# lhoangan/arap_flow

Measured on AMD Instinct MI355X. Metric: ARAP solve+warp frames/sec at 854x480 mesh, higher is better.
Workload: dtype f32; 1 GPU; configs[1]: single 854x480 DAVIS-shaped frame, single-segment mask, fd=1; schedule 19/8/400; segments_per_frame=1, fd=1, parallelism=frames sharded, no collective, grid_vertices_per_frame=409920

## Files before the change

arap_flow_amd/csrc/arap_resident.h:

```cpp
#pragma once
#include <type_traits>
#include "arap_device.h"

namespace arap {

constexpr int RES_WGS = 512;
constexpr int RES_MAX_GROUPS = 16;
constexpr int RES_THREADS = 256;
constexpr int RES_SLOTS = 9;
constexpr int RES_TILES_PER_WG = RES_SLOTS;
constexpr int RT_X = 32, RT_Y = 8;
constexpr int RES_ZX = 2 * RT_X + 2 * RT_Y;
constexpr int RES_ZG = 2 * RES_ZX;
constexpr int RES_MAX_L = 32000;
static_assert(RT_X * RT_Y == RES_THREADS && RT_Y == 2 * (RES_THREADS / 64), "one vertex per lane, two rows per wavefront");
constexpr int RES_MAX_HALO = RES_TILES_PER_WG * (2 * RT_X + 2 * RT_Y);
constexpr int RES_HALO_PER_THREAD = (RES_MAX_HALO + RES_THREADS - 1) / RES_THREADS;
constexpr int RES_MAX_TILES = RES_WGS * RES_TILES_PER_WG;
constexpr int LROW = RT_X + 2;
constexpr int LROWS = RT_Y + 2;
constexpr int LPLANE = LROW * LROWS;
constexpr int LTILE = 5 * LPLANE;
constexpr int RES_LDS_BYTES = RES_TILES_PER_WG * LTILE * 4
                              + ((RES_MAX_HALO * 8 + 15) / 16) * 16
                              + RES_TILES_PER_WG * 8 + 8 + 384
                              + RES_TILES_PER_WG * RES_ZX * 16;
static_assert(2 * ((RES_LDS_BYTES + 1279) / 1280 * 1280) <= 160 * 1024, "two workgroups per CU");
#ifndef RES_HALO_REG_SLOTS
#define RES_HALO_REG_SLOTS 8
#endif
#ifndef RES_WREG_SLOTS
#define RES_WREG_SLOTS 7
#endif
#ifndef RES_WREG_8
#define RES_WREG_8 2
#endif
#ifndef RES_WREG_9
#define RES_WREG_9 2
#endif
#ifndef RES_WREG_FIT
#define RES_WREG_FIT 6
#endif
#ifndef RES_WREG_FIT_FLAT
#define RES_WREG_FIT_FLAT 7
#endif
#ifndef RES_WREG_8_FLAT
#define RES_WREG_8_FLAT 3
#endif
#ifndef RES_WREG_9_FLAT
#define RES_WREG_9_FLAT RES_WREG_9
#endif
#ifndef RES_FIRST_LOOK
#define RES_FIRST_LOOK 5
#endif
#ifndef RES_FIRST_LOOK_2
#define RES_FIRST_LOOK_2 14
#endif
#ifndef RES_FIRST_LOOK_X
#define RES_FIRST_LOOK_X 20
#endif
#ifndef RES_OWN_LOCAL
#define RES_OWN_LOCAL 1
#endif
#ifndef RES_POLL_SLEEP
#define RES_POLL_SLEEP 1
#endif
constexpr unsigned RES_SPIN_LIMIT = 1u << 18;
#ifndef RES_GRAN_STRIDE
#define RES_GRAN_STRIDE 2
#endif
constexpr int RES_GS = RES_GRAN_STRIDE;
constexpr int RES_GRAN_UNITS = 2 * RES_WGS;
constexpr int RES_GRAN_L1 = 2 * RES_GRAN_UNITS * RES_GS;
constexpr int RES_GRAN2_STRIDE = 16;
constexpr int RES_GRAN2_GROUP = 2 * 8 * RES_GRAN2_STRIDE;
constexpr int RES_GRAN_X = RES_GRAN_L1 + 4 * RES_GRAN2_GROUP;
constexpr int RES_GRAN_PER_LAUNCH = RES_GRAN_X + RES_GRAN_L1;
#ifndef RES_FLAT_MAX_RUNS
#define RES_FLAT_MAX_RUNS 2
#endif

constexpr int RES_SUMS_ANY = 0, RES_SUMS_FLAT = 1, RES_SUMS_COUNT = 2;

struct ResWg {
    int slot;
    int rank;
    int wgs;
    int gran;
};

struct ResDev {
    const int* tilelist;
    const int* ntiles;
    const int* tilepos;
    const int* bandx0;
    unsigned long long* zx;
    int rtX, rtY;
    unsigned long long* gran;
    unsigned* err;
    const ResWg* wgmap;
    int allow_fast;
    int force_fail;
    int flat_runs;
    int nowait;
    int fuse_update;
    unsigned long long* stamps;
};

typedef __attribute__((address_space(1))) unsigned long long gu64;
typedef __attribute__((address_space(1))) unsigned gu32;

__device__ __forceinline__ int border_entry(int x, int y)
{
    return y == 0 ? x : (y == RT_Y - 1 ? RT_X + x : (x == 0 ? 2 * RT_X + y : (x == RT_X - 1 ? 2 * RT_X + RT_Y + y : -1)));
}
__device__ __forceinline__ void st_tagged(unsigned long long* p, unsigned hi , float v, bool fast)
{
    const unsigned long long g = ((unsigned long long)hi << 32) | __float_as_uint(v);
    if (fast) __hip_atomic_store(p, g, __ATOMIC_RELAXED, __HIP_MEMORY_SCOPE_WORKGROUP);
    else __hip_atomic_store(p, g, __ATOMIC_RELAXED, __HIP_MEMORY_SCOPE_AGENT);
}
typedef float v2f_t __attribute__((ext_vector_type(2)));
__device__ __forceinline__ float2 fma2(float2 a, float2 b, float2 c)
{
    const v2f_t r = __builtin_elementwise_fma((v2f_t){a.x, a.y}, (v2f_t){b.x, b.y}, (v2f_t){c.x, c.y});
    return make_float2(r.x, r.y);
}
template <int BITNO>
__device__ __forceinline__ float keep_if(unsigned f, float v)
{
    int m;
    asm("v_bfe_i32 %0, %1, %2, 1" : "=v"(m) : "v"(f), "n"(BITNO));
    return __uint_as_float(__float_as_uint(v) & (unsigned)m);
}

__device__ __forceinline__ double block_sum_uniform(double t)
{
    return __hiloint2double(__builtin_amdgcn_readlane(__double2hiint(t), 3), __builtin_amdgcn_readlane(__double2loint(t), 3));
}

__device__ __forceinline__ bool group_sum(double part, unsigned epoch, unsigned long long* gran_group, int rank,
                                          int wgs, float* bcast , unsigned* err, float& out,
                                          bool fast = false, double* out_d = nullptr, bool nowait = false,
                                          unsigned long long* tm = nullptr ,
                                          unsigned long long* tarr = nullptr )
{
    const int wave = threadIdx.x >> 6, lane = threadIdx.x & 63;
    unsigned long long c0 = 0ull, c1;
    if (wave == 0) {
        if (tm) c0 = __builtin_amdgcn_s_memtime();
        if (tarr) *tarr += __builtin_amdgcn_s_memrealtime();
        __builtin_amdgcn_s_setprio(3);
        unsigned long long* buf = gran_group + (size_t)(epoch & 1u) * wgs * RES_GS;
        if ((lane >> 1) == 1) {
            const unsigned long long bits = (unsigned long long)__double_as_longlong(part);
            const unsigned hw = lane == 2 ? (unsigned)bits : (unsigned)(bits >> 32);
            const unsigned long long gv = ((unsigned long long)epoch << 32) | hw;
            if (fast)
                __hip_atomic_store(buf + rank * RES_GS + (lane - 2), gv, __ATOMIC_RELAXED, __HIP_MEMORY_SCOPE_WORKGROUP);
            else
                __hip_atomic_store(buf + rank * RES_GS + (lane - 2), gv, __ATOMIC_RELAXED, __HIP_MEMORY_SCOPE_AGENT);
        }
        part = block_sum_uniform(part);
        double v = 0.0;
        bool ok = false;
        if (tm) { c1 = __builtin_amdgcn_s_memtime(); tm[0] += c1 - c0; c0 = c1; }
        __builtin_amdgcn_s_sleep(RES_FIRST_LOOK);
        for (unsigned spins = 0; spins < RES_SPIN_LIMIT; ++spins) {
            if (tm) tm[3] += 1;
            v = 0.0;
            bool mine_ok = true;
            for (int m = lane; m < wgs; m += 64) {
                const unsigned long long lo = __hip_atomic_load(buf + RES_GS * m, __ATOMIC_RELAXED, __HIP_MEMORY_SCOPE_AGENT);
                const unsigned long long hi =
                    __hip_atomic_load(buf + RES_GS * m + 1, __ATOMIC_RELAXED, __HIP_MEMORY_SCOPE_AGENT);
                const bool own = RES_OWN_LOCAL && m == rank;
                mine_ok = mine_ok && (own || ((unsigned)(lo >> 32) == epoch && (unsigned)(hi >> 32) == epoch));
                v += own ? part : __longlong_as_double((long long)((hi << 32) | (lo & 0xffffffffull)));
            }
            ok = __all(mine_ok) || nowait;
            if (ok) break;
            if (RES_POLL_SLEEP) __builtin_amdgcn_s_sleep(1);
        }
        if (tm) { c1 = __builtin_amdgcn_s_memtime(); tm[1] += c1 - c0; c0 = c1; asm volatile("" : "+v"(v)); }
        v = wave_sum_l63_full(v);
        if (tm) {
            asm volatile("" :: "v"(v));
            c1 = __builtin_amdgcn_s_memtime(); tm[4] += c1 - c0;
        }
        if (lane == 63) {
            *(float2*)(bcast + 2 * (epoch & 1u)) = make_float2((float)v, ok ? 1.0f : 0.0f);
            if (out_d) *out_d = v;
            if (!ok) atomicExch(err, 0xDEAD0000u | (epoch & 0xffffu));
        }
        __builtin_amdgcn_s_setprio(0);
        if (tm) { c1 = __builtin_amdgcn_s_memtime(); tm[2] += c1 - c0; c0 = c1; }
    }
    __syncthreads();
    const float2 bc = *(const float2*)(bcast + 2 * (epoch & 1u));
    out = bc.x;
    if (tm && wave == 0) {
        asm volatile("s_waitcnt lgkmcnt(0)" ::: "memory");
        tm[5] += __builtin_amdgcn_s_memtime() - c0;
    }
    return bc.y != 0.0f;
}

__device__ __forceinline__ bool group_sum_h(double part, unsigned epoch, unsigned long long* gran_group,
                                            unsigned long long* gran2 , int rank, int wgs,
                                            float* bcast, unsigned* err, float& out, bool subfast)
{
    const int wave = threadIdx.x >> 6, lane = threadIdx.x & 63;
    if (wave == 0) {
        __builtin_amdgcn_s_setprio(3);
        const int sub = rank >> 6, srank = rank & 63, nsub = wgs >> 6;
        unsigned long long* buf = gran_group + (size_t)sub * (128 * RES_GS) + (size_t)(epoch & 1u) * (64 * RES_GS);
        part = __hiloint2double(__builtin_amdgcn_readfirstlane(__double2hiint(part)),
                                __builtin_amdgcn_readfirstlane(__double2loint(part)));
        if (lane < 2) {
            const unsigned long long bits = (unsigned long long)__double_as_longlong(part);
            const unsigned hw = lane == 0 ? (unsigned)bits : (unsigned)(bits >> 32);
            const unsigned long long gv = ((unsigned long long)epoch << 32) | hw;
// ... 100 lines not shown
        v = wave_sum_l63_full(v);
        if (lane == 63) {
            *(float2*)(bcast + 2 * (epoch & 1u)) = make_float2((float)v, ok ? 1.0f : 0.0f);
            if (!ok) atomicExch(err, 0xDEAD4000u | (epoch & 0x3fffu));
        }
        __builtin_amdgcn_s_setprio(0);
    }
    __syncthreads();
    const float2 bc = *(const float2*)(bcast + 2 * (epoch & 1u));
    out = bc.x;
    return bc.y != 0.0f;
}

__device__ __forceinline__ void halo_append(bool take, unsigned short val, unsigned short* hlist, int* nhalo)
{
    const unsigned long long m = __ballot(take);
    if (m == 0ull) return;
    const int first = __builtin_ctzll(m);
    int base = 0;
    if ((int)(threadIdx.x & 63) == first) base = atomicAdd(nhalo, __popcll(m));
    base = __builtin_amdgcn_readlane(base, first);
    const int before = (int)__builtin_amdgcn_mbcnt_hi((unsigned)(m >> 32), __builtin_amdgcn_mbcnt_lo((unsigned)m, 0u));
    if (take) hlist[base + before] = val;
}

__device__ __forceinline__ double block_sum8(double v, double* wsum ,
                                             unsigned long long* tb = nullptr )
{
    static_assert(RES_THREADS / 64 == 4, "one pair sum and one DPP step add four wavefronts");
    unsigned long long c0 = 0ull, c1;
    if (tb) { c0 = __builtin_amdgcn_s_memtime(); asm volatile("" : "+v"(v)); }
    v = wave_sum_l63_full(v);
    if (tb) { asm volatile("" :: "v"(v)); c1 = __builtin_amdgcn_s_memtime(); tb[0] += c1 - c0; c0 = c1; }
    const int wave = threadIdx.x >> 6, lane = threadIdx.x & 63;
    if (lane == 63) wsum[wave] = v;
    __syncthreads();
    double t = 0.0;
    if (wave == 0) {
        const double a = wsum[lane & 3], b = wsum[(lane & 3) ^ 1];
        if (tb) { asm volatile("s_waitcnt lgkmcnt(0)" ::: "memory"); c1 = __builtin_amdgcn_s_memtime(); tb[1] += c1 - c0; c0 = c1; }
        t = dpp_add_f64_full<0x112, 0xf>(a + b);
        if (tb) { asm volatile("" :: "v"(t)); c1 = __builtin_amdgcn_s_memtime(); tb[2] += c1 - c0; }
    }
    return t;
}

template <bool STAMPS, int NS, int SUMS>
__global__ __launch_bounds__(RES_THREADS, 2) void k_pcg_resident(PlanDev pd, ResDev rd, int L)
{
    static_assert(NS >= 1 && NS <= RES_SLOTS, "slots");
    static_assert(SUMS == RES_SUMS_ANY || SUMS == RES_SUMS_FLAT, "group-sum flavour");
    constexpr bool FLAT = SUMS == RES_SUMS_FLAT;
    constexpr bool SPEND = FLAT && !STAMPS;
    constexpr int WFIT = SPEND ? RES_WREG_FIT_FLAT : RES_WREG_FIT;
    unsigned long long tA = 0, tS1 = 0, tB = 0, tS2 = 0, tU = 0, t0 = 0, t1 = 0;
    unsigned long long tm[6] = {0, 0, 0, 0, 0, 0}, tbs = 0, tzr = 0;
    unsigned long long tbp[3] = {0, 0, 0}, tarr[2] = {0, 0};
#define RES_STAMP(acc) do { if (STAMPS) { t1 = __builtin_amdgcn_s_memrealtime(); acc += t1 - t0; t0 = t1; } } while (0)
    extern __shared__ __attribute__((aligned(16))) float lds[];
    const ResWg me = rd.wgmap[blockIdx.x];
    if (me.slot < 0) return;
    const int rank = me.rank;
    if (rd.force_fail) {
        if (threadIdx.x == 0) atomicExch(rd.err, 0xDEADFFFFu);
        return;
    }
    if (__hip_atomic_load(rd.err, __ATOMIC_RELAXED, __HIP_MEMORY_SCOPE_AGENT) != 0u) return;
    const int b = me.slot;
    const int wgs = me.wgs;
    const int W = pd.W, H = pd.H;
    const size_t gb = (size_t)b * pd.N;
    const int tid = threadIdx.x, lane = tid & 63, wave = tid >> 6;
    const int lx = lane & (RT_X - 1), ly = (wave << 1) | (lane >> 5);
    unsigned short* hlist = (unsigned short*)(lds + RES_TILES_PER_WG * LTILE);
    int2* tbase = (int2*)((char*)hlist + ((RES_MAX_HALO * 8 + 15) / 16) * 16);
    float* moLUT = (float*)(tbase + RES_TILES_PER_WG + 1);
    float* bcast = moLUT + 12;
    int* nhalo = (int*)(bcast + 4);
    double* wsum = (double*)(bcast + 6);
    unsigned* nbits = (unsigned*)(wsum + 10);
    unsigned* nremote = nbits + 16;
    float4* zst = (float4*)((char*)lds + RES_LDS_BYTES - RES_TILES_PER_WG * RES_ZX * 16);
    unsigned long long* gran_group = rd.gran + me.gran;
    unsigned long long* granx_group = FLAT ? nullptr : rd.gran + RES_GRAN_X + me.gran;

    const int nt = rd.ntiles[b];
    const int tbase_n = nt / wgs, textra = nt - tbase_n * wgs;
    const int tp = tbase_n + (rank < textra ? 1 : 0);
    const int tfirst = rank * tbase_n + (rank < textra ? rank : textra);
    const int* tl = rd.tilelist + (size_t)b * RES_MAX_TILES;
    float wr2, wf2;
    {
        const Slot sl = pd.slots[b];
        wr2 = sl.wr * sl.wr;
        wf2 = sl.wf * sl.wf;
        if (tid < 10) {
            const int deg = tid % 5, fit = tid / 5;
            float dO = 0.f;
            for (int k = 0; k < deg; ++k) dO = dO + (sl.wr * sl.wr + sl.wr * sl.wr);
            if (fit) dO = fmaf(sl.wf, sl.wf, dO);
            moLUT[tid] = ginv(dO);
        }
        if (tid == 0) { *nhalo = 0; *nremote = 0u; }
        if (tid < 16) nbits[tid] = 0u;
    }

    float rx[NS], ry[NS], ra[NS];
    float dx_[NS], dy_[NS], da_[NS];
    float apx[NS], apy[NS], apa[NS];
    float ma_[NS], mo_[NS];
    unsigned fl[NS];
    int ibase[NS];
    constexpr int NWR = NS <= RES_WREG_SLOTS ? 4 : (NS == 8 ? (SPEND ? RES_WREG_8_FLAT : RES_WREG_8)
                                                            : (SPEND ? RES_WREG_9_FLAT : RES_WREG_9));
    constexpr bool WREG = NWR > 0;
    float we[WREG ? NS : 1][5];
    const int loff = lx + W * ly;

    const int cell = (ly + 1) * LROW + (lx + 1);
#define TP2(T) ((float2*)(T))
#define TCS(T) ((float2*)(T) + LPLANE)
#define TPA(T) ((T) + 4 * LPLANE)

    int org_[NS];
#pragma unroll
    for (int j = 0; j < NS; ++j) org_[j] = j < tp ? tl[tfirst + j] : -1;
    unsigned long long* const zx_b = rd.zx + (size_t)b * RES_MAX_TILES * RES_ZG;
    for (int c = tid; c < tp * RES_ZG; c += RES_THREADS)
        __hip_atomic_store(zx_b + (size_t)tfirst * RES_ZG + c, 0ull, __ATOMIC_RELAXED, __HIP_MEMORY_SCOPE_AGENT);
    float2 qC[NS], qR[NS], vR[NS], vC[NS], hR[NS], hC[NS];
    float qRa[NS], qM[NS], vRa[NS], vM[NS], hRa[NS], hM[NS];
    unsigned qF[NS], vF[NS], hF[NS];
    const int vrow = ly == 0 ? 0 : RT_Y + 1, hcol = lx == 0 ? 0 : RT_X + 1;
#pragma unroll
    for (int j = 0; j < NS; ++j) {
        qC[j] = qR[j] = vR[j] = vC[j] = hR[j] = hC[j] = make_float2(0.f, 0.f);
        qRa[j] = qM[j] = vRa[j] = vM[j] = hRa[j] = hM[j] = 0.f;
        qF[j] = vF[j] = hF[j] = 0u;
        const int org = org_[j];
        const int y0 = org / W, x0 = org - y0 * W;
        const int x = x0 + lx, y = y0 + ly;
        if (org >= 0 && x < W && y < H) {
            const size_t i = gb + (size_t)(x + W * y);
            qF[j] = pd.flags[i];
            qC[j] = pd.cs[i];
            qR[j] = pd.rO[i]; qRa[j] = pd.rA[i]; qM[j] = pd.preA[i];
            if ((ly == 0 && y0 > 0) || (ly == RT_Y - 1 && y + 1 < H)) {
                const size_t hi = ly == 0 ? i - W : i + W;
                vF[j] = pd.flags[hi]; vR[j] = pd.rO[hi]; vRa[j] = pd.rA[hi]; vM[j] = pd.preA[hi]; vC[j] = pd.cs[hi];
            }
            if ((lx == 0 && x0 > 0) || (lx == RT_X - 1 && x + 1 < W)) {
                const size_t hi = lx == 0 ? i - 1 : i + 1;
                hF[j] = pd.flags[hi]; hR[j] = pd.rO[hi]; hRa[j] = pd.rA[hi]; hM[j] = pd.preA[hi]; hC[j] = pd.cs[hi];
            }
        }
    }
    for (int c = tid; c < NS * LTILE; c += RES_THREADS) lds[c] = 0.f;
    __syncthreads();
#pragma unroll
    for (int j = 0; j < NS; ++j) {
        dx_[j] = dy_[j] = da_[j] = 0.f;
        apx[j] = apy[j] = apa[j] = 0.f;
        const int org = org_[j];
        int x0 = -1, y0 = -1;
        if (org >= 0) { y0 = org / W; x0 = org - y0 * W; }
        float* T = lds + j * LTILE;
        const bool act = (qF[j] & F_ACT) != 0u;
        rx[j] = act ? qR[j].x : 0.f; ry[j] = act ? qR[j].y : 0.f; ra[j] = act ? qRa[j] : 0.f;
        ma_[j] = act ? qM[j] : 0.f;
        mo_[j] = moLUT[__popc(qF[j] & 15u) + 5 * (int)((qF[j] >> 4) & 1u)];
        if (act) {
            TP2(T)[cell] = make_float2(mo_[j] * rx[j], mo_[j] * ry[j]);
            TCS(T)[cell] = qC[j];
            TPA(T)[cell] = ma_[j] * ra[j];
        }
        if (vF[j] & F_ACT) {
            const int hc = vrow * LROW + (lx + 1);
            const float mo = moLUT[__popc(vF[j] & 15u) + 5 * (int)((vF[j] >> 4) & 1u)];
            TP2(T)[hc] = make_float2(mo * vR[j].x, mo * vR[j].y); TCS(T)[hc] = vC[j]; TPA(T)[hc] = vM[j] * vRa[j];
        }
        if (hF[j] & F_ACT) {
            const int hc = (ly + 1) * LROW + hcol;
            const float mo = moLUT[__popc(hF[j] & 15u) + 5 * (int)((hF[j] >> 4) & 1u)];
            TP2(T)[hc] = make_float2(mo * hR[j].x, mo * hR[j].y); TCS(T)[hc] = hC[j]; TPA(T)[hc] = hM[j] * hRa[j];
        }
        fl[j] = qF[j];
        ibase[j] = __builtin_amdgcn_readfirstlane(x0 + W * y0);
        if (tid == 0) tbase[j] = make_int2(x0, y0);
    }
    float rho = read_scalar(pd.red + ((size_t)b * pd.nslots + 0) * NSHARD);
    __syncthreads();
#pragma unroll
    for (int j = 0; j < NS; ++j) {
        const unsigned f = fl[j];
        if (WREG) {
            if (NWR > 0) we[j][0] = keep_if<0>(f, wr2);
            if (NWR > 1) we[j][1] = keep_if<1>(f, wr2);
            if (NWR > 2) we[j][2] = keep_if<2>(f, wr2);
            if (NWR > 3) we[j][3] = keep_if<3>(f, wr2);
            if (NS <= WFIT) we[j][4] = keep_if<4>(f, wf2);
        }
        halo_append(ly == 0 && (f & F_E3), (unsigned short)(j * LPLANE + 0 * LROW + lx + 1), hlist, nhalo);
        halo_append(ly == RT_Y - 1 && (f & F_E2), (unsigned short)(j * LPLANE + (RT_Y + 1) * LROW + lx + 1), hlist, nhalo);
        halo_append(lx == 0 && (f & F_E1), (unsigned short)(j * LPLANE + (ly + 1) * LROW + 0), hlist, nhalo);
        halo_append(lx == RT_X - 1 && (f & F_E0), (unsigned short)(j * LPLANE + (ly + 1) * LROW + RT_X + 1), hlist, nhalo);
    }
    __syncthreads();
    const int nh = *nhalo;
    uint2* htab = (uint2*)hlist;
    constexpr bool HREG = NS <= RES_HALO_REG_SLOTS;
    uint2 hreg[RES_HALO_PER_THREAD];
    {
        uint2 e[RES_HALO_PER_THREAD];
#pragma unroll
        for (int u = 0; u < RES_HALO_PER_THREAD; ++u) {
            const int c = tid + u * RES_THREADS;
            e[u] = make_uint2(0u, 0u);
            if (c < nh) {
                const int id = hlist[c];
                const int k = id / LPLANE, rem = id - k * LPLANE;
                const int row = rem / LROW, col = rem - row * LROW;
                const int2 tb = tbase[k];
                const int gx = tb.x + col - 1, gy = tb.y + row - 1;
                e[u].y = (unsigned)(k * (LTILE / 2) + rem) | ((unsigned)(k * LTILE + 4 * LPLANE + rem) << 16);
                const int band = gy / RT_Y;
                const int kx = (gx - rd.bandx0[(size_t)b * rd.rtY + band]) / RT_X;
                const int pos = rd.tilepos[((size_t)b * rd.rtY + band) * rd.rtX + (kx < 0 ? 0 : (kx < rd.rtX ? kx : rd.rtX - 1))];
                const int nfull = textra * (tbase_n + 1);
                const int owner = pos < nfull ? pos / (tbase_n + 1) : textra + (pos - nfull) / (tbase_n > 0 ? tbase_n : 1);
                if (pos >= 0 && owner != rank) atomicOr(&nbits[(owner >> 5) & 15], 1u << (owner & 31));
                const int kxc = kx < 0 ? 0 : (kx < rd.rtX ? kx : rd.rtX - 1);
                const int lxo = gx - (rd.bandx0[(size_t)b * rd.rtY + band] + kxc * RT_X), lyo = gy - band * RT_Y;
                const int zpos = border_entry(lxo, lyo);
                (void)row; (void)col;
                e[u].x = (unsigned)((pos < 0 ? 0 : pos) * RES_ZG + 2 * zpos);
            }
        }
        __syncthreads();
#pragma unroll
        for (int u = 0; u < RES_HALO_PER_THREAD; ++u) {
            if (tid + u * RES_THREADS < RES_MAX_HALO) htab[tid + u * RES_THREADS] = e[u];
            hreg[u] = e[u];
        }
    }
    static_assert(RES_TILES_PER_WG * LTILE < 65536 && LTILE % 2 == 0, "halo table packs 16-bit cell offsets");

    unsigned offP[5], offA[5];
    {
        const int dn[5] = {0, 1, -1, LROW, -LROW};
#pragma unroll
        for (int n = 0; n < 5; ++n) {
            offP[n] = (unsigned)(cell + dn[n]) * 8u;
            offA[n] = (unsigned)(cell + dn[n]) * 4u;
            asm volatile("" : "+v"(offP[n]));
            asm volatile("" : "+v"(offA[n]));
        }
    }
    const int zent = border_entry(lx, ly);
    bool alive = true;
    float alpha_last = 0.f;
    asm volatile("s_waitcnt vmcnt(0)" ::: "memory");
    __syncthreads();
    bool fast = false, zfast = false;
    bool hier = false, subfast = false;
    bool hierx = false;
    unsigned long long* const gran2 =
        FLAT ? nullptr : rd.gran + RES_GRAN_L1 + ((((int)(blockIdx.x & 7u) - (me.rank >> 6)) >> 1) & 3) * RES_GRAN2_GROUP;
    {
        const unsigned xcc = __builtin_amdgcn_s_getreg((3 << 11) | (0 << 6) | 20) & 15u;
        float dummy;
        const double mine = (double)xcc + 65536.0 * (double)(xcc * xcc);
        alive = group_sum(mine, 1u, gran_group, rank, wgs, bcast, rd.err, dummy, false, wsum + 8);
        const double tot = wsum[8];
        const double s2 = floor(tot / 65536.0), s1 = tot - 65536.0 * s2;
        fast = rd.allow_fast && ((double)wgs * s2 == s1 * s1);
        __syncthreads();
        hier = !FLAT && !fast && wgs > 64;
        hierx = hier && (((wgs + 63) >> 6) <= 2 || ((wgs + 63) >> 6) <= rd.flat_runs);
        if (!fast && rd.allow_fast && alive) {
            if (wave == 0) {
                const unsigned long long* buf = gran_group + (size_t)1 * wgs * RES_GS;
                bool remote = false, elsewhere = false;
                for (int m = lane; m < wgs; m += 64) {
                    const bool nb = ((nbits[(m >> 5) & 15] >> (m & 31)) & 1u) != 0u;
                    const bool same_run = hier && (m >> 6) == (rank >> 6);
                    if (nb || same_run) {
                        const unsigned long long lo = __hip_atomic_load(buf + RES_GS * m, __ATOMIC_RELAXED, __HIP_MEMORY_SCOPE_AGENT);
                        const unsigned long long hi = __hip_atomic_load(buf + RES_GS * m + 1, __ATOMIC_RELAXED, __HIP_MEMORY_SCOPE_AGENT);
                        const double val = __longlong_as_double((long long)((hi << 32) | (lo & 0xffffffffull)));
                        const double q2 = floor(val / 65536.0);
                        const bool other = (unsigned)(lo >> 32) != 1u || (unsigned)(hi >> 32) != 1u ||
                                           (unsigned)(val - 65536.0 * q2) != xcc;
                        remote = remote || (nb && other);
                        elsewhere = elsewhere || (same_run && other);
                    }
                }
                const unsigned any_remote = __any(remote) ? 1u : 0u, any_elsewhere = __any(elsewhere) ? 2u : 0u;
                if (lane == 0) *nremote = any_remote | any_elsewhere;
            }
            __syncthreads();
            zfast = (*nremote & 1u) == 0u;
            subfast = !FLAT && hier && (*nremote & 2u) == 0u;
        } else {
            zfast = fast;
        }
        __syncthreads();
    }
#ifndef RES_PRIO_HI
#define RES_PRIO_HI 2
#endif
#ifndef RES_PRIO_TAIL
#define RES_PRIO_TAIL 2
#endif
#define RES_PRIO(J) { if ((J) + RES_PRIO_TAIL >= NS) __builtin_amdgcn_s_setprio(0); else __builtin_amdgcn_s_setprio(RES_PRIO_HI); }
#define RES_PRIO_END() __builtin_amdgcn_s_setprio(0);
    if (STAMPS) t0 = __builtin_amdgcn_s_memrealtime();
    for (int l = 0; l < L && alive; ++l) {
        static_assert(F_E0 == 1u && F_E1 == 2u && F_E2 == 4u && F_E3 == 8u && F_FIT == 16u && F_ACT == 32u, "bit numbers below");
        double acc = 0.0;
        float2 Lpv[2], Lcs[2], LqO[2][4], Lcn[2][4];
        float Lpa[2], LqA[2][4];
#define RES_LOAD_A(J)                                                                                  \
        {                                                                                              \
            const int s_ = (J) & 1;                                                                    \
            const char* T_ = (const char*)lds + (J) * (LTILE * 4);                                     \
            Lpv[s_] = *(const float2*)(T_ + offP[0]);                                                  \
            Lcs[s_] = *(const float2*)(T_ + offP[0] + LPLANE * 8);                                     \
            Lpa[s_] = *(const float*)(T_ + offA[0] + LPLANE * 16);                                     \
            _Pragma("unroll") for (int n_ = 0; n_ < 2; ++n_) {                                         \
                LqO[s_][n_] = *(const float2*)(T_ + offP[n_ + 1]);                                     \
                Lcn[s_][n_] = *(const float2*)(T_ + offP[n_ + 1] + LPLANE * 8);                        \
                LqA[s_][n_] = *(const float*)(T_ + offA[n_ + 1] + LPLANE * 16);                        \
            }                                                                                          \
        }
#define RES_LOAD_B(J)                                                                                  \
        {                                                                                              \
            const int s_ = (J) & 1;                                                                    \
            const char* T_ = (const char*)lds + (J) * (LTILE * 4);                                     \
            _Pragma("unroll") for (int n_ = 2; n_ < 4; ++n_) {                                         \
                LqO[s_][n_] = *(const float2*)(T_ + offP[n_ + 1]);                                     \
                Lcn[s_][n_] = *(const float2*)(T_ + offP[n_ + 1] + LPLANE * 8);                        \
                LqA[s_][n_] = *(const float*)(T_ + offA[n_ + 1] + LPLANE * 16);                        \
            }                                                                                          \
        }
        RES_LOAD_A(0)
        RES_LOAD_B(0)
#pragma unroll
        for (int j = 0; j < NS; ++j) {
            RES_PRIO(j)
            unsigned f = fl[j];
            asm volatile("" : "+v"(f));
            const int sj = j & 1;
            if (j + 1 < NS) RES_LOAD_A(j + 1)
            __builtin_amdgcn_sched_barrier(0);
            {
                const float2 pv = Lpv[sj];
                const float2 csv = Lcs[sj];
                const float pa_ = Lpa[sj];
                const float ci = csv.x, si = csv.y;
                const float2 pa2 = make_float2(pa_, pa_);
                float2 axy = make_float2(0.f, 0.f);
                float aa = 0.f;
#define RES_EDGE(BITNO, E, NQX, NQY, NHX, NHY, QX, QY)                                                 \
                {                                                                                      \
                    const float2 qO = LqO[sj][E], cn2 = Lcn[sj][E];                                    \
                    const float qA = LqA[sj][E];                                                       \
                    const float cn = cn2.x, sn = cn2.y;                                                \
                    const float w = (BITNO < NWR) ? we[WREG ? j : 0][BITNO] : keep_if<BITNO>(f, wr2);  \
                    const float2 e = pv - qO;                                                          \
                    const float2 t = fma2(make_float2(NQX, NQY), pa2, e);                              \
                    const float2 u = fma2(make_float2(NHX, NHY), make_float2(qA, qA), e + t);          \
                    axy = fma2(make_float2(w, w), u, axy);                                             \
                    aa = fmaf(-w, fmaf(QX, t.x, (QY) * t.y), aa);                                      \
                    (void)cn; (void)sn;                                                                \
                }
                RES_EDGE(0, 0,     -si,  ci,   -sn,  cn,    si, -ci)
                RES_EDGE(1, 1,      si, -ci,    sn, -cn,   -si,  ci)
                __builtin_amdgcn_sched_barrier(0);
                if (j + 1 < NS) RES_LOAD_B(j + 1)
                __builtin_amdgcn_sched_barrier(0);
                RES_EDGE(2, 2,     -ci, -si,   -cn, -sn,    ci,  si)
                RES_EDGE(3, 3,      ci,  si,    cn,  sn,   -ci, -si)
#undef RES_EDGE
                {
                    const float wf = (WREG && NS <= WFIT) ? we[WREG ? j : 0][4] : keep_if<4>(f, wf2);
                    axy = fma2(make_float2(wf, wf), pv, axy);
                }
                const float ax = axy.x, ay = axy.y;
                apx[j] = ax; apy[j] = ay; apa[j] = aa;
                acc += (double)dot3(pv.x, pv.y, pa_, ax, ay, aa);
            }
            __builtin_amdgcn_sched_barrier(0);
        }
#undef RES_LOAD_A
#undef RES_LOAD_B
        float sigma;
        RES_PRIO_END()
        RES_STAMP(tA);
        {
            const unsigned long long cb = STAMPS ? __builtin_amdgcn_s_memtime() : 0ull;
            const double bs = block_sum8(acc, wsum, STAMPS ? tbp : nullptr);
            if (STAMPS) tbs += __builtin_amdgcn_s_memtime() - cb;
            alive = (!FLAT && hierx) ? group_sum_x(block_sum_uniform(bs), 2u * l + 2u, gran_group, granx_group, rank, wgs, bcast, rd.err, sigma, subfast)
                  : (!FLAT && hier)  ? group_sum_h(block_sum_uniform(bs), 2u * l + 2u, gran_group, gran2, rank, wgs, bcast, rd.err, sigma, subfast)
                          : group_sum(bs, 2u * l + 2u, gran_group, rank, wgs, bcast, rd.err, sigma, fast, nullptr, rd.nowait != 0,
                                      STAMPS ? tm : nullptr, STAMPS ? tarr : nullptr);
        }
        asm volatile("" : "+v"(sigma));
        if (!alive) break;
        RES_STAMP(tS1);
        float alpha = 0.f;
        if (sigma > 0.f) alpha = rho / sigma;
        acc = 0.0;
        const unsigned ztag = 2u * l + 3u;
#pragma unroll
        for (int j = 0; j < NS; ++j) {
            RES_PRIO(j)
            unsigned f = fl[j];
            asm volatile("" : "+v"(f));
            const float mo = mo_[j], ma = ma_[j];
            rx[j] = fmaf(-alpha, apx[j], rx[j]);
            ry[j] = fmaf(-alpha, apy[j], ry[j]);
            ra[j] = fmaf(-alpha, apa[j], ra[j]);
            const float zx = mo * rx[j], zy = mo * ry[j], za = ma * ra[j];
            if (zent >= 0) {
                zst[j * RES_ZX + zent] = make_float4(zx, zy, za, zy);
            }
            acc += (double)keep_if<5>(f, dot3(zx, zy, za, rx[j], ry[j], ra[j]));
            __builtin_amdgcn_sched_barrier(0);
        }
        float rhoNew;
        RES_PRIO_END()
        RES_STAMP(tB);
        {
            const unsigned long long cb = STAMPS ? __builtin_amdgcn_s_memtime() : 0ull;
            const double bs = block_sum8(acc, wsum, STAMPS ? tbp : nullptr);
            if (STAMPS) tbs += __builtin_amdgcn_s_memtime() - cb;
            if (wave != 0) {
                unsigned long long* const out = zx_b + (size_t)tfirst * RES_ZG;
                const float2* const st2 = (const float2*)zst;
                const unsigned sh = (tid & 1) ? 16u : 0u;
                static_assert(((RES_THREADS - 64) & 1) == 0, "a thread keeps the parity of its granules");
                if (zfast) {
                    for (int g = tid - 64; g < tp * RES_ZG; g += RES_THREADS - 64) {
                        const float2 v = st2[g];
                        st_tagged(out + g, (ztag << 16) | ((__float_as_uint(v.y) >> sh) & 0xffffu), v.x, true);
                    }
                } else {
                    for (int g = tid - 64; g < tp * RES_ZG; g += RES_THREADS - 64) {
                        const float2 v = st2[g];
                        st_tagged(out + g, (ztag << 16) | ((__float_as_uint(v.y) >> sh) & 0xffffu), v.x, false);
                    }
                }
            }
            alive = (!FLAT && hierx) ? group_sum_x(block_sum_uniform(bs), 2u * l + 3u, gran_group, granx_group, rank, wgs, bcast, rd.err, rhoNew, subfast)
                  : (!FLAT && hier)  ? group_sum_h(block_sum_uniform(bs), 2u * l + 3u, gran_group, gran2, rank, wgs, bcast, rd.err, rhoNew, subfast)
                          : group_sum(bs, 2u * l + 3u, gran_group, rank, wgs, bcast, rd.err, rhoNew, fast, nullptr, rd.nowait != 0,
                                      STAMPS ? tm : nullptr, STAMPS ? tarr + 1 : nullptr);
        }
        unsigned long long hg[RES_HALO_PER_THREAD][2];
        unsigned hpk_[HREG ? 1 : RES_HALO_PER_THREAD];
#define RES_HPK(U) (HREG ? hreg[U].y : hpk_[HREG ? 0 : (U)])
#pragma unroll
        for (int u = 0; u < RES_HALO_PER_THREAD; ++u) {
            hg[u][0] = hg[u][1] = (unsigned long long)ztag << 48;
            if (tid + u * RES_THREADS < nh) {
                const unsigned gi = HREG ? hreg[u].x : htab[tid + u * RES_THREADS].x;
                const unsigned long long* q_ = (const unsigned long long*)((const char*)zx_b + (size_t)(gi * 8u));
#pragma unroll
                for (int c = 0; c < 2; ++c) hg[u][c] = __hip_atomic_load(q_ + c, __ATOMIC_RELAXED, __HIP_MEMORY_SCOPE_AGENT);
            }
        }
        if (!alive) break;
        RES_STAMP(tS2);
        float beta = 0.f;
        if (rho > 0.f) beta = rhoNew / rho;
        rho = rhoNew;
        if (l + 1 == L) { alpha_last = alpha; break; }
        float2 hp2[RES_HALO_PER_THREAD];
        float hpa[RES_HALO_PER_THREAD];
        {
            float2 Up[NS];
            float Ua[NS];
#pragma unroll
            for (int j = 0; j < NS; ++j) {
                const char* T_ = (const char*)lds + j * (LTILE * 4);
                Up[j] = *(const float2*)(T_ + offP[0]);
                Ua[j] = *(const float*)(T_ + offA[0] + LPLANE * 16);
            }
            __builtin_amdgcn_sched_barrier(0);
#pragma unroll
            for (int j = 0; j < NS; ++j) {
                RES_PRIO(j)
                char* T_ = (char*)lds + j * (LTILE * 4);
                const float mo = mo_[j], ma = ma_[j];
                const float zx = mo * rx[j], zy = mo * ry[j], za = ma * ra[j];
                dx_[j] = fmaf(alpha, Up[j].x, dx_[j]);
                dy_[j] = fmaf(alpha, Up[j].y, dy_[j]);
                da_[j] = fmaf(alpha, Ua[j], da_[j]);
                *(float2*)(T_ + offP[0]) = make_float2(fmaf(beta, Up[j].x, zx), fmaf(beta, Up[j].y, zy));
                *(float*)(T_ + offA[0] + LPLANE * 16) = fmaf(beta, Ua[j], za);
            }
        }
        __builtin_amdgcn_sched_barrier(0);
        {
#pragma unroll
            for (int u = 0; u < RES_HALO_PER_THREAD; ++u) {
                hp2[u] = make_float2(0.f, 0.f); hpa[u] = 0.f;
                if (!HREG) hpk_[u] = 0u;
                if (tid + u * RES_THREADS < nh) {
                    if (!HREG) hpk_[u] = htab[tid + u * RES_THREADS].y;
                    hp2[u] = *(const float2*)((const char*)lds + (RES_HPK(u) & 0xffffu) * 8u);
                    hpa[u] = *(const float*)((const char*)lds + (RES_HPK(u) >> 16) * 4u);
                }
            }
        }
#pragma unroll
        for (int j = 0; j < NS; ++j)
            if (HREG) asm volatile("" : "+v"(dx_[j]), "+v"(dy_[j]), "+v"(da_[j]));
        __builtin_amdgcn_sched_barrier(0);
        {
            bool fresh = true;
#pragma unroll
            for (int u = 0; u < RES_HALO_PER_THREAD; ++u)
#pragma unroll
                for (int c = 0; c < 2; ++c) fresh = fresh && (unsigned)(hg[u][c] >> 48) == ztag;
            if (!__all(fresh) && !rd.nowait) {
                for (unsigned spins = 0; spins < RES_SPIN_LIMIT; ++spins) {
                    if (STAMPS) tzr += 1;
                    fresh = true;
#pragma unroll
                    for (int u = 0; u < RES_HALO_PER_THREAD; ++u) {
                        if (tid + u * RES_THREADS < nh) {
                            const unsigned gi = HREG ? hreg[u].x : htab[tid + u * RES_THREADS].x;
                            const unsigned long long* q_ = (const unsigned long long*)((const char*)zx_b + (size_t)(gi * 8u));
#pragma unroll
                            for (int c = 0; c < 2; ++c) {
                                hg[u][c] = __hip_atomic_load(q_ + c, __ATOMIC_RELAXED, __HIP_MEMORY_SCOPE_AGENT);
                                fresh = fresh && (unsigned)(hg[u][c] >> 48) == ztag;
                            }
                        }
                    }
                    if (__all(fresh)) break;
                    __builtin_amdgcn_s_sleep(1);
                }
                if (!fresh) atomicExch(rd.err, 0xDEAD0000u | (ztag & 0xffffu));
            }
        }
#pragma unroll
        for (int u = 0; u < RES_HALO_PER_THREAD; ++u) {
            const float2 hz2_ = make_float2(__uint_as_float((unsigned)hg[u][0]),
                                            __uint_as_float(((unsigned)(hg[u][0] >> 32) & 0xffffu) | ((unsigned)(hg[u][1] >> 32) << 16)));
            const float hz1_ = __uint_as_float((unsigned)hg[u][1]);
            if (tid + u * RES_THREADS < nh) {
                float2* P = (float2*)((char*)lds + (RES_HPK(u) & 0xffffu) * 8u);
                float* A = (float*)((char*)lds + (RES_HPK(u) >> 16) * 4u);
                *P = make_float2(fmaf(beta, hp2[u].x, hz2_.x), fmaf(beta, hp2[u].y, hz2_.y));
                *A = fmaf(beta, hpa[u], hz1_);
            }
        }
        RES_PRIO_END()
        __syncthreads();
        RES_STAMP(tU);
    }
    if (STAMPS && tid == 0) {
        unsigned long long* o = rd.stamps + (size_t)blockIdx.x * 16;
        o[8] = tbs; o[9] = tm[0]; o[10] = tm[1]; o[11] = tm[2]; o[12] = tm[3]; o[13] = tzr;
        o[0] = tA; o[1] = tS1; o[2] = tB; o[3] = tS2; o[4] = tU; o[5] = (unsigned long long)tp; { unsigned pc = 0; for (int q = 0; q < 16; ++q) pc += __popc(nbits[q]); o[6] = (unsigned long long)nh | ((unsigned long long)pc << 32) | ((unsigned long long)*nremote << 48); } o[7] = (fast ? 1ull : 0ull) | (zfast ? 2ull : 0ull) | (hier ? 4ull : 0ull) | (subfast ? 8ull : 0ull);
        unsigned long long* q = rd.stamps + (size_t)RES_WGS * 16 + (size_t)blockIdx.x * 16;
        q[0] = tbp[0]; q[1] = tbp[1]; q[2] = tbp[2]; q[3] = tm[4]; q[4] = tm[5]; q[5] = tarr[0]; q[6] = tarr[1];
        q[7] = (unsigned long long)__builtin_amdgcn_s_getreg((31 << 11) | (0 << 6) | 4) |
               ((unsigned long long)(__builtin_amdgcn_s_getreg((3 << 11) | (0 << 6) | 20) & 15u) << 32);
        q[8] = (unsigned long long)tp; q[9] = (unsigned long long)nh; q[10] = (unsigned long long)tp * RES_ZG;
        q[11] = (unsigned long long)rank | ((unsigned long long)wgs << 16) | ((unsigned long long)b << 32); q[12] = (unsigned long long)L;
    }
    if (!alive) return;
    if (L > 0) {
#pragma unroll
        for (int j = 0; j < NS; ++j) {
            const char* T_ = (const char*)lds + j * (LTILE * 4);
            const float2 p2 = *(const float2*)(T_ + offP[0]);
            const float pa1 = *(const float*)(T_ + offA[0] + LPLANE * 16);
            dx_[j] = fmaf(alpha_last, p2.x, dx_[j]);
            dy_[j] = fmaf(alpha_last, p2.y, dy_[j]);
            da_[j] = fmaf(alpha_last, pa1, da_[j]);
        }
    }
    int lo = loff;
    asm volatile("" : "+v"(lo));
    if (rd.fuse_update) {
        const Slot sl = pd.slots[b];
        float2 o_[NS];
        float a_[NS];
#pragma unroll
        for (int j = 0; j < NS; ++j) {
            o_[j] = make_float2(0.f, 0.f); a_[j] = 0.f;
            if (fl[j] & F_ACT) { const int i = ibase[j] + lo; o_[j] = sl.O[i]; a_[j] = sl.A[i]; }
        }
#pragma unroll
        for (int j = 0; j < NS; ++j) {
            if (fl[j] & F_ACT) {
                const int i = ibase[j] + lo;
                float2 o = o_[j];
                o.x = o.x + dx_[j];
                o.y = o.y + dy_[j];
                const float a = a_[j] + da_[j];
                sl.O[i] = o;
                sl.A[i] = a;
                pd.cs[gb + i] = sincos_spec(a);
            }
        }
        return;
    }
#pragma unroll
    for (int j = 0; j < NS; ++j) {
        const unsigned f = fl[j];
        if (f & F_ACT) {
            const int i = ibase[j] + lo;
            pd.deltaO[gb + i] = make_float2(dx_[j], dy_[j]);
            pd.deltaA[gb + i] = da_[j];
        }
    }
}

#undef RES_STAMP
#undef RES_HPK
#undef RES_PRIO
#undef RES_PRIO_END
#undef TP2
#undef TCS
#undef TPA

}
```

arap_flow_amd/csrc/host_resident.h:

```cpp
#pragma once

typedef void (*ResidentKernel)(PlanDev, ResDev, int);
template <bool STAMPS, int SUMS, int... NS>
static const void* resident_kernel_of(int ns, std::integer_sequence<int, NS...>)
{
    static const ResidentKernel table[] = {k_pcg_resident<STAMPS, NS + 1, SUMS>...};
    return (const void*)table[ns - 1];
}
static const void* resident_kernel(bool stamps, int ns, int sums)
{
    if (ns < 1) ns = 1;
    if (ns > RES_SLOTS) ns = RES_SLOTS;
    const auto slots = std::make_integer_sequence<int, RES_SLOTS>();
    if (sums == RES_SUMS_FLAT)
        return stamps ? resident_kernel_of<true, RES_SUMS_FLAT>(ns, slots) : resident_kernel_of<false, RES_SUMS_FLAT>(ns, slots);
    return stamps ? resident_kernel_of<true, RES_SUMS_ANY>(ns, slots) : resident_kernel_of<false, RES_SUMS_ANY>(ns, slots);
}
static const char* resident_sums_name(int sums) { return sums == RES_SUMS_FLAT ? "flat" : "any"; }

static void plan_enable_resident(Opt_Plan* p)
{
    Opt_State* st = p->st;
    const Knobs knobs = read_knobs();
    p->knob_res_groups = knobs.res_groups;
// ... 301 lines not shown
                    if (kind[b] == MEDIUM) {
                        for (int j = 0; j < XW; ++j)
                            map[(size_t)set * RES_WGS + (size_t)j * 8 + x] = ResWg{b, j, wgs_of[b], gran_of[b]};
                        continue;
                    }
                    const bool first = x == 0 || owner[k - 1] != b;
                    if (!first) continue;
                    for (int q = 0; q < width[b]; ++q)
                        for (int j = 0; j < XW; ++j)
                            map[(size_t)set * RES_WGS + (size_t)j * 8 + x + q] = ResWg{b, q * XW + j, wgs_of[b], gran_of[b]};
                    continue;
                }
                int j = 0;
                for (int b : order) {
                    if (kind[b] == WIDE || bin_of[b] != (int)k) continue;
                    take_gran(b);
                    const int r0 = kind[b] == MEDIUM ? XW : 0;
                    for (int r = 0; r < part_w[b]; ++r, ++j)
                        map[(size_t)set * RES_WGS + (size_t)j * 8 + x] = ResWg{b, r0 + r, wgs_of[b], gran_of[b]};
                }
            }
            inflight = count > inflight ? count : inflight;
        }
    }
    if (map_out) map_out->swap(map);
    if (inflight_out) *inflight_out = inflight;
    return nsets;
}

static int resident_launch_sums(const ResWg* map, bool force_any)
{
    if (force_any) return RES_SUMS_ANY;
    for (int i = 0; i < RES_WGS; ++i)
        if (map[i].slot >= 0 && map[i].wgs > RES_WGS / 8) return RES_SUMS_ANY;
    return RES_SUMS_FLAT;
}

static bool plan_resident_pack(Opt_Plan* p)
{
    std::vector<ResWg> map;
    const int nsets = resident_deal(p->h_ntiles.data(), p->nb, p->knob_res_groups, &map, &p->res_inflight);
    std::vector<int> ns(nsets, 1);
    for (size_t i = 0; i < map.size(); ++i)
        if (map[i].slot >= 0) {
            const int t = (p->h_ntiles[map[i].slot] + map[i].wgs - 1) / map[i].wgs;
            int& m = ns[i / RES_WGS];
            m = t > m ? t : m;
        }
    if (p->knob_res_ns > 0)
        for (int& m : ns) m = std::max(m, std::min(p->knob_res_ns, (int)RES_SLOTS));
    std::vector<int> sums(nsets, RES_SUMS_ANY);
    for (int set = 0; set < nsets; ++set)
        sums[set] = resident_launch_sums(map.data() + (size_t)set * RES_WGS, p->knob_res_sums_any);
    const bool same = nsets == p->res_sets && ns == p->res_ns && sums == p->res_sums && map.size() == p->h_wgmap.size() &&
                      memcmp(map.data(), p->h_wgmap.data(), map.size() * sizeof(ResWg)) == 0;
    if (same) return false;
    p->h_wgmap.swap(map);
    p->res_ns.swap(ns);
    p->res_sums.swap(sums);
    p->res_sets = nsets;
    return true;
}

static void plan_upload_wgmap(Opt_Plan* p)
{
    Opt_State* st = p->st;
    if (p->hole_pending) {
        std::vector<ResWg> holed = p->h_wgmap;
        for (ResWg& w : holed)
            if (w.slot >= 0 && w.wgs > 1 && w.rank == w.wgs - 1) { w = ResWg{-1, 0, 0, 0}; break; }
        HC(hipStreamSynchronize(st->stream));
        HC(hipMemcpy(p->d_wgmap, holed.data(), holed.size() * sizeof(ResWg), hipMemcpyHostToDevice));
        p->hole_pending = false;
    } else {
        memcpy(p->pin_wgmap, p->h_wgmap.data(), p->h_wgmap.size() * sizeof(ResWg));
        HC(hipMemcpyAsync(p->d_wgmap, p->pin_wgmap, p->h_wgmap.size() * sizeof(ResWg), hipMemcpyHostToDevice,
                          st->stream));
    }
}

static bool plan_resident_failed(Opt_Plan* p)
{
    if (!p->res_capable || p->res_launches == 0) return false;
    unsigned e = 0;
    HC(hipMemcpyAsync(&e, p->rd.err, sizeof(e), hipMemcpyDeviceToHost, p->st->stream));
    HC(hipStreamSynchronize(p->st->stream));
    if (e == 0) return false;
    Opt_State* st = p->st;
    fprintf(stderr, "arapopt: resident PCG kernel gave up at a group wait (code 0x%08x); is the GPU shared? "
                    "Falling back to the two-kernel path for the next %d solve calls.\n", e, st->res_backoff);
    st->resident_failed = true;
    st->res_cooldown = st->res_backoff;
    st->res_backoff = st->res_backoff >= 1024 ? 1024 : 2 * st->res_backoff;
    HC(hipMemsetAsync((void*)p->rd.err, 0, sizeof(unsigned), st->stream));
    HC(hipStreamSynchronize(st->stream));
    p->h_wgmap.clear();
    p->res_sets = 0;
    return true;
}

static void plan_check_resident_error(Opt_Plan* p)
{
    if (plan_resident_failed(p)) {
        fprintf(stderr, "arapopt: resident PCG failure detected after results were consumed\n");
        exit(3);
    }
// ... 2 lines not shown
```

Baseline: 30.63 frames/s.

## Keep search direction in registers, single-sweep group sum, retune weight-register knobs

Adds a register-resident copy of the PCG search direction p and preconditioned residual z for slot counts up to seven. The matvec reads p from registers instead of LDS, and the p update is done in registers before being written back to LDS for neighbours. The flat group-sum flavour now polls peers with one lane per workgroup in a single sweep, and the host aborts if a group larger than 64 is dealt to it. The change also raises the weight-register slot knobs, pins weights in registers with empty asm, and sets RES_MAX_GROUPS to RES_WGS. All of this raises register pressure, which risks spills or lower occupancy at two workgroups per CU.

```diff
diff --git a/arap_flow_amd/csrc/arap_resident.h b/arap_flow_amd/csrc/arap_resident.h
--- a/arap_flow_amd/csrc/arap_resident.h
+++ b/arap_flow_amd/csrc/arap_resident.h
@@ -5,7 +5,7 @@
 namespace arap {
 
 constexpr int RES_WGS = 512;
-constexpr int RES_MAX_GROUPS = 16;
+constexpr int RES_MAX_GROUPS = RES_WGS;
 constexpr int RES_THREADS = 256;
 constexpr int RES_SLOTS = 9;
 constexpr int RES_TILES_PER_WG = RES_SLOTS;
@@ -33,19 +33,31 @@
 #define RES_WREG_SLOTS 7
 #endif
 #ifndef RES_WREG_8
-#define RES_WREG_8 2
+#define RES_WREG_8 4
 #endif
 #ifndef RES_WREG_9
-#define RES_WREG_9 2
+#define RES_WREG_9 4
 #endif
 #ifndef RES_WREG_FIT
-#define RES_WREG_FIT 6
+#define RES_WREG_FIT 9
 #endif
 #ifndef RES_WREG_FIT_FLAT
-#define RES_WREG_FIT_FLAT 7
+#define RES_WREG_FIT_FLAT 9
+#endif
+#ifndef RES_WPIN
+#define RES_WPIN 1
+#endif
+#ifndef RES_PREG_SLOTS
+#define RES_PREG_SLOTS 7
+#endif
+#ifndef RES_PREG_SLOTS_FLAT
+#define RES_PREG_SLOTS_FLAT 7
+#endif
+#ifndef RES_SWEEP1
+#define RES_SWEEP1 1
 #endif
 #ifndef RES_WREG_8_FLAT
-#define RES_WREG_8_FLAT 3
+#define RES_WREG_8_FLAT 4
 #endif
 #ifndef RES_WREG_9_FLAT
 #define RES_WREG_9_FLAT RES_WREG_9
@@ -139,6 +151,7 @@
     return __hiloint2double(__builtin_amdgcn_readlane(__double2hiint(t), 3), __builtin_amdgcn_readlane(__double2loint(t), 3));
 }
 
+template <bool ONE = false>
 __device__ __forceinline__ bool group_sum(double part, unsigned epoch, unsigned long long* gran_group, int rank,
                                           int wgs, float* bcast , unsigned* err, float& out,
                                           bool fast = false, double* out_d = nullptr, bool nowait = false,
@@ -166,8 +179,22 @@
         bool ok = false;
         if (tm) { c1 = __builtin_amdgcn_s_memtime(); tm[0] += c1 - c0; c0 = c1; }
         __builtin_amdgcn_s_sleep(RES_FIRST_LOOK);
+        const bool own1 = RES_OWN_LOCAL && lane == rank;
+        const bool look = ONE && lane < wgs && !own1;
+        const double idle = own1 ? part : 0.0;
+        const unsigned long long* const q1 = buf + RES_GS * ((ONE && lane < wgs) ? lane : 0);
         for (unsigned spins = 0; spins < RES_SPIN_LIMIT; ++spins) {
             if (tm) tm[3] += 1;
+            if (ONE) {
+                const unsigned long long lo = __hip_atomic_load(q1, __ATOMIC_RELAXED, __HIP_MEMORY_SCOPE_AGENT);
+                const unsigned long long hi = __hip_atomic_load(q1 + 1, __ATOMIC_RELAXED, __HIP_MEMORY_SCOPE_AGENT);
+                const bool late = look && ((unsigned)(lo >> 32) != epoch || (unsigned)(hi >> 32) != epoch);
+                v = look ? __longlong_as_double((long long)((hi << 32) | (lo & 0xffffffffull))) : idle;
+                ok = !__any(late) || nowait;
+                if (ok) break;
+                if (RES_POLL_SLEEP) __builtin_amdgcn_s_sleep(1);
+                continue;
+            }
             v = 0.0;
             bool mine_ok = true;
             for (int m = lane; m < wgs; m += 64) {
@@ -374,6 +401,8 @@
     static_assert(SUMS == RES_SUMS_ANY || SUMS == RES_SUMS_FLAT, "group-sum flavour");
     constexpr bool FLAT = SUMS == RES_SUMS_FLAT;
     constexpr bool SPEND = FLAT && !STAMPS;
+    constexpr bool ONE_TRIP = FLAT && RES_SWEEP1 != 0;
+    constexpr bool PREG = NS <= (FLAT ? RES_PREG_SLOTS_FLAT : RES_PREG_SLOTS);
     constexpr int WFIT = SPEND ? RES_WREG_FIT_FLAT : RES_WREG_FIT;
     unsigned long long tA = 0, tS1 = 0, tB = 0, tS2 = 0, tU = 0, t0 = 0, t1 = 0;
     unsigned long long tm[6] = {0, 0, 0, 0, 0, 0}, tbs = 0, tzr = 0;
@@ -431,11 +460,15 @@
     float dx_[NS], dy_[NS], da_[NS];
     float apx[NS], apy[NS], apa[NS];
     float ma_[NS], mo_[NS];
+    float2 pxy[PREG ? NS : 1];
+    float pal[PREG ? NS : 1];
+    float zx_[PREG ? NS : 1], zy_[PREG ? NS : 1], za_[PREG ? NS : 1];
     unsigned fl[NS];
     int ibase[NS];
     constexpr int NWR = NS <= RES_WREG_SLOTS ? 4 : (NS == 8 ? (SPEND ? RES_WREG_8_FLAT : RES_WREG_8)
                                                             : (SPEND ? RES_WREG_9_FLAT : RES_WREG_9));
     constexpr bool WREG = NWR > 0;
+    constexpr bool WPIN = WREG && RES_WPIN != 0;
     float we[WREG ? NS : 1][5];
     const int loff = lx + W * ly;
 
@@ -491,10 +524,16 @@
         rx[j] = act ? qR[j].x : 0.f; ry[j] = act ? qR[j].y : 0.f; ra[j] = act ? qRa[j] : 0.f;
         ma_[j] = act ? qM[j] : 0.f;
         mo_[j] = moLUT[__popc(qF[j] & 15u) + 5 * (int)((qF[j] >> 4) & 1u)];
+        const float2 p0 = make_float2(mo_[j] * rx[j], mo_[j] * ry[j]);
+        const float pa0 = ma_[j] * ra[j];
         if (act) {
-            TP2(T)[cell] = make_float2(mo_[j] * rx[j], mo_[j] * ry[j]);
+            TP2(T)[cell] = p0;
             TCS(T)[cell] = qC[j];
-            TPA(T)[cell] = ma_[j] * ra[j];
+            TPA(T)[cell] = pa0;
+        }
+        if (PREG) {
+            pxy[j] = act ? p0 : make_float2(0.f, 0.f);
+            pal[j] = act ? pa0 : 0.f;
         }
         if (vF[j] & F_ACT) {
             const int hc = vrow * LROW + (lx + 1);
@@ -592,7 +631,7 @@
         const unsigned xcc = __builtin_amdgcn_s_getreg((3 << 11) | (0 << 6) | 20) & 15u;
         float dummy;
         const double mine = (double)xcc + 65536.0 * (double)(xcc * xcc);
-        alive = group_sum(mine, 1u, gran_group, rank, wgs, bcast, rd.err, dummy, false, wsum + 8);
+        alive = group_sum<ONE_TRIP>(mine, 1u, gran_group, rank, wgs, bcast, rd.err, dummy, false, wsum + 8);
         const double tot = wsum[8];
         const double s2 = floor(tot / 65536.0), s1 = tot - 65536.0 * s2;
         fast = rd.allow_fast && ((double)wgs * s2 == s1 * s1);
@@ -639,6 +678,13 @@
     if (STAMPS) t0 = __builtin_amdgcn_s_memrealtime();
     for (int l = 0; l < L && alive; ++l) {
         static_assert(F_E0 == 1u && F_E1 == 2u && F_E2 == 4u && F_E3 == 8u && F_FIT == 16u && F_ACT == 32u, "bit numbers below");
+        if (WPIN) {
+#pragma unroll
+            for (int j = 0; j < NS; ++j)
+#pragma unroll
+                for (int e_ = 0; e_ < 5; ++e_)
+                    if (e_ < NWR || (e_ == 4 && NS <= WFIT)) asm volatile("" : "+v"(we[WREG ? j : 0][e_]));
+        }
         double acc = 0.0;
         float2 Lpv[2], Lcs[2], LqO[2][4], Lcn[2][4];
         float Lpa[2], LqA[2][4];
@@ -646,9 +692,9 @@
         {                                                                                              \
             const int s_ = (J) & 1;                                                                    \
             const char* T_ = (const char*)lds + (J) * (LTILE * 4);                                     \
-            Lpv[s_] = *(const float2*)(T_ + offP[0]);                                                  \
+            if (!PREG) Lpv[s_] = *(const float2*)(T_ + offP[0]);                                       \
             Lcs[s_] = *(const float2*)(T_ + offP[0] + LPLANE * 8);                                     \
-            Lpa[s_] = *(const float*)(T_ + offA[0] + LPLANE * 16);                                     \
+            if (!PREG) Lpa[s_] = *(const float*)(T_ + offA[0] + LPLANE * 16);                          \
             _Pragma("unroll") for (int n_ = 0; n_ < 2; ++n_) {                                         \
                 LqO[s_][n_] = *(const float2*)(T_ + offP[n_ + 1]);                                     \
                 Lcn[s_][n_] = *(const float2*)(T_ + offP[n_ + 1] + LPLANE * 8);                        \
@@ -676,9 +722,9 @@
             if (j + 1 < NS) RES_LOAD_A(j + 1)
             __builtin_amdgcn_sched_barrier(0);
             {
-                const float2 pv = Lpv[sj];
+                const float2 pv = PREG ? pxy[PREG ? j : 0] : Lpv[sj];
                 const float2 csv = Lcs[sj];
-                const float pa_ = Lpa[sj];
+                const float pa_ = PREG ? pal[PREG ? j : 0] : Lpa[sj];
                 const float ci = csv.x, si = csv.y;
                 const float2 pa2 = make_float2(pa_, pa_);
                 float2 axy = make_float2(0.f, 0.f);
@@ -725,7 +771,7 @@
             if (STAMPS) tbs += __builtin_amdgcn_s_memtime() - cb;
             alive = (!FLAT && hierx) ? group_sum_x(block_sum_uniform(bs), 2u * l + 2u, gran_group, granx_group, rank, wgs, bcast, rd.err, sigma, subfast)
                   : (!FLAT && hier)  ? group_sum_h(block_sum_uniform(bs), 2u * l + 2u, gran_group, gran2, rank, wgs, bcast, rd.err, sigma, subfast)
-                          : group_sum(bs, 2u * l + 2u, gran_group, rank, wgs, bcast, rd.err, sigma, fast, nullptr, rd.nowait != 0,
+                          : group_sum<ONE_TRIP>(bs, 2u * l + 2u, gran_group, rank, wgs, bcast, rd.err, sigma, fast, nullptr, rd.nowait != 0,
                                       STAMPS ? tm : nullptr, STAMPS ? tarr : nullptr);
         }
         asm volatile("" : "+v"(sigma));
@@ -745,6 +791,7 @@
             ry[j] = fmaf(-alpha, apy[j], ry[j]);
             ra[j] = fmaf(-alpha, apa[j], ra[j]);
             const float zx = mo * rx[j], zy = mo * ry[j], za = ma * ra[j];
+            if (PREG) { zx_[j] = zx; zy_[j] = zy; za_[j] = za; }
             if (zent >= 0) {
                 zst[j * RES_ZX + zent] = make_float4(zx, zy, za, zy);
             }
@@ -777,7 +824,7 @@
             }
             alive = (!FLAT && hierx) ? group_sum_x(block_sum_uniform(bs), 2u * l + 3u, gran_group, granx_group, rank, wgs, bcast, rd.err, rhoNew, subfast)
                   : (!FLAT && hier)  ? group_sum_h(block_sum_uniform(bs), 2u * l + 3u, gran_group, gran2, rank, wgs, bcast, rd.err, rhoNew, subfast)
-                          : group_sum(bs, 2u * l + 3u, gran_group, rank, wgs, bcast, rd.err, rhoNew, fast, nullptr, rd.nowait != 0,
+                          : group_sum<ONE_TRIP>(bs, 2u * l + 3u, gran_group, rank, wgs, bcast, rd.err, rhoNew, fast, nullptr, rd.nowait != 0,
                                       STAMPS ? tm : nullptr, STAMPS ? tarr + 1 : nullptr);
         }
         unsigned long long hg[RES_HALO_PER_THREAD][2];
@@ -801,7 +848,20 @@
         if (l + 1 == L) { alpha_last = alpha; break; }
         float2 hp2[RES_HALO_PER_THREAD];
         float hpa[RES_HALO_PER_THREAD];
-        {
+        if (PREG) {
+#pragma unroll
+            for (int j = 0; j < (PREG ? NS : 0); ++j) {
+                RES_PRIO(j)
+                char* T_ = (char*)lds + j * (LTILE * 4);
+                dx_[j] = fmaf(alpha, pxy[j].x, dx_[j]);
+                dy_[j] = fmaf(alpha, pxy[j].y, dy_[j]);
+                da_[j] = fmaf(alpha, pal[j], da_[j]);
+                pxy[j] = make_float2(fmaf(beta, pxy[j].x, zx_[j]), fmaf(beta, pxy[j].y, zy_[j]));
+                pal[j] = fmaf(beta, pal[j], za_[j]);
+                *(float2*)(T_ + offP[0]) = pxy[j];
+                *(float*)(T_ + offA[0] + LPLANE * 16) = pal[j];
+            }
+        } else {
             float2 Up[NS];
             float Ua[NS];
 #pragma unroll
@@ -901,8 +961,8 @@
 #pragma unroll
         for (int j = 0; j < NS; ++j) {
             const char* T_ = (const char*)lds + j * (LTILE * 4);
-            const float2 p2 = *(const float2*)(T_ + offP[0]);
-            const float pa1 = *(const float*)(T_ + offA[0] + LPLANE * 16);
+            const float2 p2 = PREG ? pxy[PREG ? j : 0] : *(const float2*)(T_ + offP[0]);
+            const float pa1 = PREG ? pal[PREG ? j : 0] : *(const float*)(T_ + offA[0] + LPLANE * 16);
             dx_[j] = fmaf(alpha_last, p2.x, dx_[j]);
             dy_[j] = fmaf(alpha_last, p2.y, dy_[j]);
             da_[j] = fmaf(alpha_last, pa1, da_[j]);
diff --git a/arap_flow_amd/csrc/host_resident.h b/arap_flow_amd/csrc/host_resident.h
--- a/arap_flow_amd/csrc/host_resident.h
+++ b/arap_flow_amd/csrc/host_resident.h
@@ -377,6 +377,12 @@
     std::vector<int> sums(nsets, RES_SUMS_ANY);
     for (int set = 0; set < nsets; ++set)
         sums[set] = resident_launch_sums(map.data() + (size_t)set * RES_WGS, p->knob_res_sums_any);
+    for (size_t i = 0; i < map.size(); ++i)
+        if (map[i].slot >= 0 && sums[i / RES_WGS] == RES_SUMS_FLAT && map[i].wgs > 64) {
+            fprintf(stderr, "arapopt: a group of %d workgroups was dealt to a launch of the flat group-sum flavour, "
+                            "whose one-trip sweep covers 64\n", map[i].wgs);
+            exit(3);
+        }
     const bool same = nsets == p->res_sets && ns == p->res_ns && sums == p->res_sums && map.size() == p->h_wgmap.size() &&
                       memcmp(map.data(), p->h_wgmap.data(), map.size() * sizeof(ResWg)) == 0;
     if (same) return false;
```

Result: faster. 32.05 frames/s, median of 6 (+4.6%).
